# heracles-ec/heracles

Hardware: AMD Instinct MI355X
Metric: map->Cl pairs/sec + mixing-matrix build sec, nside=4096 lmax=6144 (higher is better)
Workload: dtype f64

## Files before the change

### heracles_amd/csrc/hx_fft_core.h

```cpp
#pragma once
#ifdef __HIPCC__
#include <hip/hip_runtime.h>
#define HX_HD __host__ __device__ __forceinline__
#else
#include <cmath>
#define HX_HD inline
struct double2 {
    double x, y;
};
#endif

namespace hxfft {

HX_HD double2 mk(double a, double b)
{
    double2 r;
    r.x = a;
    r.y = b;
    return r;
}
HX_HD double2 cadd(double2 a, double2 b) { return mk(a.x + b.x, a.y + b.y); }
HX_HD double2 csub(double2 a, double2 b) { return mk(a.x - b.x, a.y - b.y); }
HX_HD double2 cmul(double2 a, double2 b) { return mk(a.x * b.x - a.y * b.y, a.x * b.y + a.y * b.x); }
HX_HD double2 cmulc(double2 a, double2 b)
// ... 89 lines not shown
#endif
    for (int s = 0; s < K; ++s) {
        const int half = R >> (s + 1);
#ifdef __HIPCC__
#pragma unroll
#endif
        for (int b = 0; b < R; b += 2 * half)
#ifdef __HIPCC__
#pragma unroll
#endif
            for (int jj = 0; jj < half; ++jj) {
                const double2 u = x[b + jj], v = x[b + jj + half];
                x[b + jj] = cadd(u, v);
                x[b + jj + half] = rot16(csub(u, v), jj * (8 / half));
            }
    }
}
template <int K>
HX_HD void dit_inv_regs(double2 *x)
{
    constexpr int R = 1 << K;
#ifdef __HIPCC__
#pragma unroll
#endif
    for (int s = K - 1; s >= 0; --s) {
        const int half = R >> (s + 1);
#ifdef __HIPCC__
#pragma unroll
#endif
        for (int b = 0; b < R; b += 2 * half)
#ifdef __HIPCC__
#pragma unroll
#endif
            for (int jj = 0; jj < half; ++jj) {
                const double2 u = x[b + jj], v = rot16c(x[b + jj + half], jj * (8 / half));
                x[b + jj] = cadd(u, v);
                x[b + jj + half] = csub(u, v);
            }
    }
}

template <int K, class TW>
HX_HD void dif_pass_butterfly(double2 *buf, int i, int h, TW tw, int twN)
{
    constexpr int R = 1 << K;
    const int t = i & (h - 1), p = ((i - t) << K) + t;
    double2 x[R];
#ifdef __HIPCC__
#pragma unroll
#endif
    for (int j = 0; j < R; ++j) x[j] = buf[lds_slot(p + j * h)];
    dif_regs<K>(x);
    if (h > 1 && t) apply_tw_powers<K, false>(x, tw[t * (twN / (R * h))]);
#ifdef __HIPCC__
#pragma unroll
#endif
    for (int j = 0; j < R; ++j) buf[lds_slot(p + j * h)] = x[j];
}
template <int K, class TW>
HX_HD void dit_inv_pass_butterfly(double2 *buf, int i, int h, TW tw, int twN)
{
    constexpr int R = 1 << K;
    const int t = i & (h - 1), p = ((i - t) << K) + t;
    double2 x[R];
#ifdef __HIPCC__
#pragma unroll
#endif
    for (int j = 0; j < R; ++j) x[j] = buf[lds_slot(p + j * h)];
    if (h > 1 && t) apply_tw_powers<K, true>(x, tw[t * (twN / (R * h))]);
    dit_inv_regs<K>(x);
#ifdef __HIPCC__
#pragma unroll
#endif
    for (int j = 0; j < R; ++j) buf[lds_slot(p + j * h)] = x[j];
}

HX_HD int fft_sched_np(int p) { return p <= 0 ? 0 : (p - (p < 4 ? p : 4) + 3) / 4 + 1; }
HX_HD int fft_sched_k(int p, int a)
{
    const int last = p < 4 ? p : 4, rest = p - last, nfront = (rest + 3) / 4;
    return a < nfront ? rest / nfront + (a < rest % nfront ? 1 : 0) : last;
}

HX_HD double2 dif4_combine(double2 z0, double2 z1, double2 z2, double2 z3, int r)
{
    switch (r & 3) {
    case 0: return cadd(cadd(z0, z1), cadd(z2, z3));
    case 1: return cadd(csub(z0, z2), mul_mi(csub(z1, z3)));
    case 2: return cadd(csub(z0, z1), csub(z2, z3));
    default: return cadd(csub(z0, z2), mul_pi(csub(z1, z3)));
    }
}

HX_HD unsigned mod_by_inv(unsigned x, unsigned d, double inv)
{
    const int q = (int)((double)x * inv);
    int r = (int)x - q * (int)d;
    if (r < 0) r += (int)d;
    if (r >= (int)d) r -= (int)d;
    return (unsigned)r;
}

HX_HD unsigned load_phase_num(unsigned j, unsigned r, unsigned n, bool bluestein)
{
    unsigned long long q = (unsigned long long)j * r;
    if (bluestein) q += 2ull * j * j;
    return (unsigned)(q % (4ull * n));
}

HX_HD unsigned chirp_num(unsigned k, unsigned n)
{
    return (unsigned)(((unsigned long long)k * k) % (2ull * n));
}

}
```

### heracles_amd/csrc/hx_ring_fft.hip

```cpp
#include <algorithm>
#include <type_traits>

#include "hx_sht_common.h"


namespace hx {
__global__ __launch_bounds__(512) void k_init_bhat(PlanDev P, const int *__restrict__ rp_list,
                                                   double2 *__restrict__ bhat)
{
    extern __shared__ double2 buf[];
    const int rp = rp_list[blockIdx.x];
    const int n = P.nsub[rp];
    const int M = fft_size_for(n);
    for (int j = threadIdx.x; j < lds_fft_slots(M); j += blockDim.x) buf[j] = make_double2(0.0, 0.0);
    __syncthreads();
    for (int j = threadIdx.x; j < n; j += blockDim.x) {
        double2 c = expipi((double)chirp_num(j, n) / (double)n);
        buf[lds_slot(j)] = c;
        if (j) buf[lds_slot(M - j)] = c;
    }
    __syncthreads();
    lds_fft_dif(buf, M, P.tw, P.twN);
    double2 *out = bhat + P.bhat_off[rp];
    for (int e = threadIdx.x; e < M; e += blockDim.x) out[M >= 16 ? (e & 15) * (M >> 4) + (e >> 4) : e] = buf[lds_slot(e)];
}

__host__ __device__ inline int ring_ph_hi(int M) { return (4 * M) / 64 + 1; }
constexpr int RING_NTMAX = 512;
constexpr int RING_FB = 8;

template <int MODE, bool WSYM = false>
__global__ __launch_bounds__(RING_NTMAX) void k_ring_subdft(PlanDev P, const RingDesc *__restrict__ desc, int nrings, int nb, int Mclass,
                                                            const double *__restrict__ maps,
                                                            const double *__restrict__ pixw,
                                                            const double2 *__restrict__ zin,
                                                            double2 *__restrict__ Y, double *__restrict__ pixout = nullptr,
                                                            const double *__restrict__ ref = nullptr)
{
    extern __shared__ double2 buf[];
    __shared__ double2 tw_hi[TW_HI_MAX], tw_lo[64];
    double2 *ph_hi = buf + lds_fft_slots(Mclass), *ph_lo = ph_hi + ring_ph_hi(Mclass);
    const int nt = blockDim.x;
    const int nitems = ((nrings + 7) >> 3) * nb * 32;
    const TwFactored twf = load_tw_factored(tw_hi, tw_lo, P.tw, P.twN);
    int tid = threadIdx.x;
    auto ring_of = [&](int item) __attribute__((always_inline)) { return ((item >> 5) / nb) * 8 + (item & 7); };
    RingDesc cur = RingDesc{0, 0, 0, 1, 0};
    if ((int)blockIdx.x < nitems && ring_of(blockIdx.x) < nrings) cur = desc[ring_of(blockIdx.x)];
    for (int item = blockIdx.x; item < nitems; item += gridDim.x) {
        const int r = (item >> 3) & 3, set = item >> 5;
        const int ring = ring_of(item), c = set % nb;
        const int itn = item + gridDim.x, ringn = itn < nitems ? ring_of(itn) : nrings;
        const bool nextv = ringn < nrings;
        if (ring >= nrings) {
            if (nextv) cur = desc[ringn];
            continue;
        }
        const int n = cur.n;
        const long long sN = cur.sN, sS = cur.sS;
        const int M = fft_size_for(n), MP = lds_fft_slots(M);
        const bool blu = M != n;
        const int p = ilog2(M);
        const double2 *bh = P.bhat + cur.bhat_off;
        const double inv = 1.0 / M, inv4n = 0.25 / (double)n;
        asm volatile("; item" : "+v"(tid));
        const bool haveS = sS >= 0, odd = r & 1, pw = MODE == 0 && !WSYM && pixw != nullptr;
        constexpr bool wsym = MODE == 0 && WSYM;
        const double sg = (r & 2) ? -1.0 : 1.0;
        const double *mpN = maps + (long long)c * P.npix + sN, *mpS = maps + (long long)c * P.npix + (haveS ? sS : sN);
        const double *pwN = pixw + sN, *pwS = pixw + (haveS ? sS : sN);
        const double2 *zp = zin + (long long)c * P.ny + sN;
        double2 z[RING_FB][4];
        struct __attribute__((aligned(8))) Pair { double x, y; };
        Pair wsy[RING_FB / 2];
        auto load_batch_t = [&](auto WIDEC, int u0) __attribute__((always_inline)) {
            constexpr bool WIDE = decltype(WIDEC)::value;
#pragma unroll
            for (int u = 0; u < RING_FB; u += 2) {
                const int j = 2 * (tid + ((u0 + u) >> 1) * nt);
                const bool tail = WIDE && j == n - 1;
                const int jj = tail ? n - 2 : (j + 1 < n ? j : 0);
                wsy[u >> 1] = Pair{1.0, 1.0};
                if (MODE == 0 && wsym && WIDE) wsy[u >> 1] = *reinterpret_cast<const Pair *>(pwN + jj);
#pragma unroll
                for (int q = 0; q < 4; ++q) {
                    const int i = jj + q * n;
                    if (MODE == 0) {
                        Pair fn, fs;
                        if (WIDE) {
                            fn = *reinterpret_cast<const Pair *>(mpN + i);
                            fs = *reinterpret_cast<const Pair *>(mpS + i);
                            if (!wsym && pw) {
                                const Pair wn = *reinterpret_cast<const Pair *>(pwN + i), ws = *reinterpret_cast<const Pair *>(pwS + i);
                                fn.x *= wn.x; fn.y *= wn.y; fs.x *= ws.x; fs.y *= ws.y;
                            }
                            z[u][q] = make_double2(fn.x, fn.y);
                            z[u + 1][q] = make_double2(fs.x, fs.y);
                        } else {
                            fn.x = fn.y = mpN[q]; fs.x = fs.y = mpS[q];
                            if (pw || wsym) { fn.x *= pwN[q]; fs.x *= pwS[q]; fn.y = fn.x; fs.y = fs.x; }
                            z[u][q] = make_double2(fn.x, haveS ? fs.x : 0.0);
                            z[u + 1][q] = make_double2(fn.y, haveS ? fs.y : 0.0);
                        }
                    } else {
                        const int i0 = (j < n ? j : 0) + q * n, i1 = (j + 1 < n ? j + 1 : 0) + q * n;
                        z[u][q] = zp[i0];
                        z[u + 1][q] = zp[i1];
                    }
                }
            }
        };
        auto load_batch = [&](int u0) __attribute__((always_inline)) {
            if (n >= 2) load_batch_t(std::true_type{}, u0);
            else load_batch_t(std::false_type{}, u0);
        };
        auto finish_batch = [&](int u0) __attribute__((always_inline)) {
            if (MODE != 0 || n < 2) return;
#pragma unroll
            for (int u = 0; u < RING_FB; u += 2) {
                const int j = 2 * (tid + ((u0 + u) >> 1) * nt);
                const bool tail = j == n - 1;
                const Pair w = wsy[u >> 1];
#pragma unroll
                for (int q = 0; q < 4; ++q) {
                    const double2 rn = z[u][q], rs = z[u + 1][q];
                    const double nx = wsym ? rn.x * w.x : rn.x, ny = wsym ? rn.y * w.y : rn.y;
                    const double sx = wsym ? rs.x * w.x : rs.x, sy = wsym ? rs.y * w.y : rs.y;
                    z[u][q] = make_double2(tail ? ny : nx, haveS ? (tail ? sy : sx) : 0.0);
                    z[u + 1][q] = make_double2(ny, haveS ? sy : 0.0);
                }
            }
        };
        load_batch(0);
        int4 nd0 = make_int4(0, 0, 0, 0), nd1 = nd0;
        if (nextv) {
            const int4 *dp = reinterpret_cast<const int4 *>(desc + ringn) + (tid >> 30);
            nd0 = dp[0];
            nd1 = dp[1];
        }
        auto lds_barrier = []() __attribute__((always_inline)) {
            __builtin_amdgcn_s_waitcnt(0xc07f);
            __builtin_amdgcn_s_barrier();
        };
        lds_barrier();
        for (int a = tid; a <= (4 * n) >> 6; a += nt) ph_hi[a] = expipi(-(double)(a << 6) / (2.0 * n));
        if (tid < 64) ph_lo[tid] = expipi(-(double)tid / (2.0 * n));
        lds_barrier();
        auto phase = [&](unsigned q) __attribute__((always_inline)) {
            return cmul(ph_hi[q >> 6], ph_lo[q & 63]);
        };
        {
            for (int u0 = 0;;) {
                finish_batch(u0);
#pragma unroll
                for (int u = 0; u < RING_FB; ++u) {
                    const int j = 2 * (tid + ((u0 + u) >> 1) * nt) + (u & 1);
                    const double2 e0 = odd ? csub(z[u][0], z[u][2]) : cadd(z[u][0], z[u][2]);
                    const double2 e1 = odd ? mul_mi(csub(z[u][1], z[u][3])) : cadd(z[u][1], z[u][3]);
                    const double2 t = make_double2(fma(sg, e1.x, e0.x), fma(sg, e1.y, e0.y));
                    const unsigned jc = j < n ? j : 0;
                    const unsigned qn = blu ? mod_by_inv(jc * (unsigned)r + 2u * jc * jc, 4u * (unsigned)n, inv4n) : jc * (unsigned)r;
                    buf[j < n ? lds_slot(j) : MP - 1] = cmul(t, phase(qn));
                }
                u0 += RING_FB;
                if (u0 * nt >= n) break;
                load_batch(u0);
            }
            if (blu)
                for (int j = n + tid; j < M; j += nt) buf[lds_slot(j)] = make_double2(0.0, 0.0);
        }
        __syncthreads();
        if (nextv) {
            auto sc = [](int v) __attribute__((always_inline)) { return __builtin_amdgcn_readfirstlane(v); };
            cur.sN = ((long long)sc(nd0.y) << 32) | (unsigned)sc(nd0.x);
            cur.sS = ((long long)sc(nd0.w) << 32) | (unsigned)sc(nd0.z);
            cur.bhat_off = ((long long)sc(nd1.y) << 32) | (unsigned)sc(nd1.x);
            cur.n = sc(nd1.z);
            cur.rp = sc(nd1.w);
        }
        double2 *out = Y + (long long)c * P.ny + sN + (long long)r * n;
        double *pxN = nullptr, *pxS = nullptr;
        const double *rfN = nullptr, *rfS = nullptr;
        if (MODE == 1 && pixout) {
            pxN = pixout + (long long)c * P.npix + sN + r;
            pxS = pixout + (long long)c * P.npix + (haveS ? sS : sN) + r;
            if (ref) { rfN = ref + (long long)c * P.npix + sN + r; rfS = ref + (long long)c * P.npix + (haveS ? sS : sN) + r; }
        }
        const int kdrop0 = MODE == 0 ? (P.lmax - r) / 4 + 1 : n, kdrop1 = (4 * n - P.lmax - r + 3) / 4;
        auto emit = [&](int k, double2 v) __attribute__((always_inline)) {
            if (MODE == 0 && k >= kdrop0 && k < kdrop1) return;
            if (MODE == 1 && pxN) {
                double fn = v.x, fs = -v.y;
                if (rfN) { fn = rfN[4 * k] - fn; fs = rfS[4 * k] - fs; }
                pxN[4 * k] = fn;
                if (haveS) pxS[4 * k] = fs;
            } else {
                out[k] = v;
            }
        };
        if (!blu) {
            lds_fft_dif(buf, M, twf, P.twN);
            for (int k = tid; k < n; k += nt) emit(k, buf[lds_slot(bitrev(k, p))]);
            continue;
        }
        if (M >= 16) {
            double2 bq[16];
            const int nbf = M >> 4;
#pragma unroll
            for (int j = 0; j < 16; ++j) bq[j] = bh[j * nbf + (tid < nbf ? tid : 0)];
            lds_fft_dif(buf, M, twf, P.twN, tid, nt, true);
#pragma unroll 1
            for (int i = tid; i < nbf; i += nt) {
                double2 x[16];
#pragma unroll
                for (int j = 0; j < 16; ++j) x[j] = buf[lds_slot(16 * i) + j];
                dif_regs<4>(x);
#pragma unroll
                for (int j = 0; j < 16; ++j) {
                    x[j] = cmul(x[j], bq[j]);
                }
                if (i + nt < nbf) {
#pragma unroll
                    for (int j = 0; j < 16; ++j) bq[j] = bh[j * nbf + i + nt];
                }
                dit_inv_regs<4>(x);
#pragma unroll
                for (int j = 0; j < 16; ++j) buf[lds_slot(16 * i) + j] = x[j];
            }
            __syncthreads();
            lds_fft_dit_inv(buf, M, twf, P.twN, tid, nt, true);
        } else {
            lds_fft_dif(buf, M, twf, P.twN, tid, nt);
            for (int j = tid; j < M; j += nt) buf[lds_slot(j)] = cmul(buf[lds_slot(j)], bh[j]);
            __syncthreads();
            lds_fft_dit_inv(buf, M, twf, P.twN, tid, nt);
        }
        for (int k = tid; k < n; k += nt)
            emit(k, cscale(cmul(buf[lds_slot(k)], phase(2u * mod_by_inv((unsigned)k * (unsigned)k, 2u * (unsigned)n, 2.0 * inv4n))), inv));
    }
}

template <int MODE, bool WSYM = false>
__global__ __launch_bounds__(RING_NTMAX) void k_ring_pairfft(PlanDev P, const RingDesc *__restrict__ desc, int nrings, int nb, int M,
                                                             const double *__restrict__ maps, const double *__restrict__ pixw,
                                                             const double2 *__restrict__ zin, double2 *__restrict__ Y,
                                                             double *__restrict__ pixout = nullptr, const double *__restrict__ ref = nullptr)
{
    extern __shared__ double2 buf[];
    __shared__ double2 tw_hi[TW_HI_MAX], tw_lo[64];
    const int MP = lds_fft_slots(M), n = M, p = ilog2(M);
    double2 *ph_hi = buf + 2 * MP, *ph_lo = ph_hi + ring_ph_hi(M);
    const int nt = blockDim.x, nh = nt >> 1;
    const int nitems = ((nrings + 7) >> 3) * nb * 16;
    const TwFactored twf = load_tw_factored(tw_hi, tw_lo, P.tw, P.twN);
    int tid = threadIdx.x;
    for (int a = tid; a <= (4 * n) >> 6; a += nt) ph_hi[a] = expipi(-(double)(a << 6) / (2.0 * n));
    if (tid < 64) ph_lo[tid] = expipi(-(double)tid / (2.0 * n));
    __syncthreads();
    auto phase = [&](unsigned q) __attribute__((always_inline)) { return cmul(ph_hi[q >> 6], ph_lo[q & 63]); };
    auto ring_of = [&](int item) __attribute__((always_inline)) { return ((item >> 4) / nb) * 8 + (item & 7); };
    auto comp_of = [&](int item) __attribute__((always_inline)) { return (item >> 4) % nb; };
    RingDesc cur = RingDesc{0, 0, 0, 1, 0};
    if ((int)blockIdx.x < nitems && ring_of(blockIdx.x) < nrings) cur = desc[ring_of(blockIdx.x)];
    struct __attribute__((aligned(8))) Pair { double x, y; };
    double2 z[RING_FB][4];
    Pair wsy[RING_FB / 2];
    const bool pw = MODE == 0 && !WSYM && pixw != nullptr;
    constexpr bool wsym = MODE == 0 && WSYM;
    auto request = [&](auto U0C, const RingDesc &d, int c) __attribute__((always_inline)) {
        constexpr int U0 = decltype(U0C)::value;
        const bool hS = d.sS >= 0;
        const double *mpN = maps + (long long)c * P.npix + d.sN, *mpS = maps + (long long)c * P.npix + (hS ? d.sS : d.sN);
        const double *pwN = pixw + d.sN, *pwS = pixw + (hS ? d.sS : d.sN);
        const double2 *zp = zin + (long long)c * P.ny + d.sN;
#pragma unroll
        for (int u = U0; u < U0 + RING_FB / 2; u += 2) {
            const int j = 2 * (tid + (u >> 1) * nt), jj = j + 1 < n ? j : 0;
            wsy[u >> 1] = Pair{1.0, 1.0};
            if (MODE == 0 && wsym) wsy[u >> 1] = *reinterpret_cast<const Pair *>(pwN + jj);
#pragma unroll
            for (int q = 0; q < 4; ++q) {
                const int i = jj + q * n;
                if (MODE == 0) {
                    Pair fn = *reinterpret_cast<const Pair *>(mpN + i), fs = *reinterpret_cast<const Pair *>(mpS + i);
                    if (!wsym && pw) {
                        const Pair wn = *reinterpret_cast<const Pair *>(pwN + i), ws = *reinterpret_cast<const Pair *>(pwS + i);
                        fn.x *= wn.x; fn.y *= wn.y; fs.x *= ws.x; fs.y *= ws.y;
                    }
                    z[u][q] = make_double2(fn.x, fn.y);
                    z[u + 1][q] = make_double2(fs.x, fs.y);
                } else {
                    z[u][q] = zp[i];
                    z[u + 1][q] = zp[i + 1];
                }
            }
        }
    };
    auto finish = [&](bool hS) __attribute__((always_inline)) {
        if (MODE != 0) return;
#pragma unroll
        for (int u = 0; u < RING_FB; u += 2) {
            const Pair w = wsy[u >> 1];
#pragma unroll
            for (int q = 0; q < 4; ++q) {
                const double2 rn = z[u][q], rs = z[u + 1][q];
                const double nx = wsym ? rn.x * w.x : rn.x, ny = wsym ? rn.y * w.y : rn.y;
                const double sx = wsym ? rs.x * w.x : rs.x, sy = wsym ? rs.y * w.y : rs.y;
                z[u][q] = make_double2(nx, hS ? sx : 0.0);
                z[u + 1][q] = make_double2(ny, hS ? sy : 0.0);
            }
        }
    };
    using H0 = std::integral_constant<int, 0>;
// ... 144 lines not shown
            *o = add ? cadd(*o, v) : v;
        }
    };
    auto input = [&](int r, int j) __attribute__((always_inline)) {
        const double2 t = dif4_combine(z_at(j, 0), z_at(j, 1), z_at(j, 2), z_at(j, 3), r);
        const unsigned qn = load_phase_num(j, r, n, !plain);
        return qn ? cmul(t, expipi(-(double)qn / (2.0 * n))) : t;
    };
    for (int r = 0; r < 4; ++r) {
        if (plain) {
            __syncthreads();
#pragma unroll 4
            for (int u = 0; u < SPLIT_JMAX; ++u) {
                const int j = threadIdx.x + u * blockDim.x;
                if (j < n) buf[lds_slot(j)] = input(r, j);
            }
            __syncthreads();
            lds_fft_dif(buf, n, twf, P.twN);
            const int pbits = ilog2(n);
            for (int k = threadIdx.x; k < n; k += blockDim.x) emit(r, k, buf[lds_slot(bitrev(k, pbits))], false);
            continue;
        }
        for (int half = 0; half < 2; ++half) {
            __syncthreads();
#pragma unroll 4
            for (int u = 0; u < SPLIT_JMAX; ++u) {
                const int j = threadIdx.x + u * blockDim.x;
                if (j < C) {
                    double2 v = make_double2(0.0, 0.0);
                    if (j < n) {
                        v = input(r, j);
                        if (half) v = cmul(v, twf[j]);
                    }
                    buf[lds_slot(j)] = v;
                }
            }
            __syncthreads();
            lds_fft_dif(buf, C, twf, P.twN);
            for (int j = threadIdx.x; j < C; j += blockDim.x) buf[lds_slot(j)] = cmul(buf[lds_slot(j)], bh[half * C + j]);
            __syncthreads();
            lds_fft_dit_inv(buf, C, twf, P.twN);
#pragma unroll 4
            for (int u = 0; u < SPLIT_JMAX; ++u) {
                const int k = threadIdx.x + u * blockDim.x;
                if (k < n) {
                    double2 y = buf[lds_slot(k)];
                    if (half) y = cmulc(y, twf[k]);
                    emit(r, k, cscale(cmul(y, expipi(-(double)chirp_num(k, n) / (double)n)), inv), half != 0);
                }
            }
        }
    }
}

__global__ __launch_bounds__(256) void k_pixw_symmetry(PlanDev P, const double *__restrict__ pixw, int *__restrict__ flag)
{
    const int rp = blockIdx.x, n = P.nsub[rp];
    const long long sN = P.startN[rp], sS = P.startS[rp];
    bool ok = true;
    for (int j = threadIdx.x; j < n; j += blockDim.x) {
        const double w = pixw[sN + j];
#pragma unroll
        for (int q = 1; q < 4; ++q) ok = ok && pixw[sN + j + (long long)q * n] == w;
        if (sS >= 0) {
#pragma unroll
            for (int q = 0; q < 4; ++q) ok = ok && pixw[sS + j + (long long)q * n] == w;
        }
    }
    if (!ok) *flag = 0;
}

}

using namespace hx;

static int g_lds_fft_cap = 8192;
extern "C" int hx_set_max_lds_fft(int points)
{
    if (points < 16 || points > 8192 || (points & (points - 1))) return fail(HX_ERR_ARG, "hx_set_max_lds_fft: a power of two in [16, 8192]");
    g_lds_fft_cap = points;
    return HX_OK;
}

static size_t ring_class_lds(int M, bool pair) { return ((pair ? 2 : 1) * (size_t)lds_fft_slots(M) + ring_ph_hi(M) + 64) * sizeof(double2); }

static bool ring_class_is_pair(int n, int M, int cap) { return M == n && M >= 16 && M <= cap && ring_class_lds(M, true) + 4096 <= 160 * 1024; }

int hx::ring_fft_plan_init(hx_plan *pl, const std::vector<int> &nsub, const std::vector<long long> &sN, const std::vector<long long> &sS)
{
    const int cap = g_lds_fft_cap;
    std::map<std::pair<int, int>, std::vector<int>> byM;
    bool plain_beyond_cap = false;
    for (int rp = pl->nrp - 1; rp >= 0; --rp) {
        const int M = fft_size_for(nsub[rp]);
        byM[{M, ring_class_is_pair(nsub[rp], M, cap) ? -1 : 0}].push_back(rp);
        plain_beyond_cap = plain_beyond_cap || (M > cap && M == nsub[rp]);
    }
    const int maxM = byM.rbegin()->first.first;
    if (maxM > 2 * cap || plain_beyond_cap) return fail(HX_ERR_UNSUPPORTED, "hx_plan_create: nside=%d needs an in-LDS FFT of %d points (limit %d, %d for Bluestein rings); unsupported", pl->nside, maxM, cap, 2 * cap);
    pl->fft_cap = cap;
    pl->lds_fft = (size_t)lds_fft_slots(std::min(maxM, cap)) * sizeof(double2);
    for (auto it = byM.rbegin(); it != byM.rend(); ++it) {
        pl->fft_classes.push_back({it->first.first, (int)pl->h_fft_rp_list.size(), (int)it->second.size(), it->first.second});
        pl->h_fft_rp_list.insert(pl->h_fft_rp_list.end(), it->second.begin(), it->second.end());
    }
    HX_TRY(upload(pl->fft_rp_list, pl->h_fft_rp_list));
    std::vector<long long> boff(pl->nrp, -1);
    std::vector<int> blu_list, blu_split;
    long long btot = 0;
    std::map<int, long long> off_of_n;
    for (int rp = 0; rp < pl->nrp; ++rp) {
        int n = nsub[rp], M = fft_size_for(n);
        if (M == n) continue;
        auto it = off_of_n.find(n);
        if (it == off_of_n.end()) {
            it = off_of_n.emplace(n, btot).first;
            btot += M;
            (M > cap ? blu_split : blu_list).push_back(rp);
        }
        boff[rp] = it->second;
    }
    HX_TRY(upload(pl->bhat_off, boff));
    std::vector<RingDesc> desc;
    for (int rp : pl->h_fft_rp_list) desc.push_back(RingDesc{sN[rp], sS[rp], boff[rp], nsub[rp], rp});
    HX_TRY(upload(pl->fft_desc, desc));
    HX_TRY(pl->bhat.alloc(sizeof(double2) * std::max<long long>(btot, 1)));
    const void *const init_kernels[] = {(const void *)k_init_bhat, (const void *)k_init_bhat_split};
    const void *const ring_kernels[] = {(const void *)k_ring_subdft<0, false>,  (const void *)k_ring_subdft<0, true>,  (const void *)k_ring_subdft<1, false>,
                                        (const void *)k_ring_pairfft<0, false>, (const void *)k_ring_pairfft<0, true>, (const void *)k_ring_pairfft<1, false>,
                                        (const void *)k_ring_subdft_split<0>,   (const void *)k_ring_subdft_split<1>};
    for (const void *k : init_kernels) (void)hipFuncSetAttribute(k, hipFuncAttributeMaxDynamicSharedMemorySize, 160 * 1024);
    for (const void *k : ring_kernels) (void)hipFuncSetAttribute(k, hipFuncAttributeMaxDynamicSharedMemorySize, 156 * 1024);
    HX_HIP(hipGetLastError());
    hipStream_t st = rt().stream;
    if (!blu_list.empty()) {
        DevBuf d_list;
        HX_TRY(upload(d_list, blu_list));
        hipLaunchKernelGGL(k_init_bhat, dim3((unsigned)blu_list.size()), dim3(512), pl->lds_fft, st, pl->dev(),
                           d_list.as<int>(), pl->bhat.as<double2>());
        (void)hipStreamSynchronize(st);
    }
    if (!blu_split.empty()) {
        DevBuf d_list;
        HX_TRY(upload(d_list, blu_split));
        hipLaunchKernelGGL(k_init_bhat_split, dim3((unsigned)blu_split.size()), dim3(std::min(512, std::max(64, cap / 16))), (size_t)lds_fft_slots(cap) * sizeof(double2), st,
                           pl->dev(), d_list.as<int>(), cap, pl->bhat.as<double2>());
        (void)hipStreamSynchronize(st);
    }
    return HX_OK;
}

struct RingIO { const double *maps, *pixw; const double2 *zin; double2 *Y; double *pixout; const double *ref; };

template <auto KERNEL>
static void launch_ring_class(hx_plan *pl, const hx_plan::FftClass &c, int nb, const RingIO &io)
{
    const int k = c.big < 0 ? 2 : 1;
    const int threads = std::min(RING_NTMAX, k * std::max(64, c.M / 16));
    const size_t lds = ring_class_lds(c.M, k == 2);
    const int per_cu = (int)std::max<size_t>(1, std::min<size_t>(512 / threads, (160 * 1024) / (lds + 3 * 1024 + 256)));
    const long long items = ((long long)c.count + 7) / 8 * nb * (32 / k);
    const unsigned groups = (unsigned)std::min<long long>(items, (long long)rt().cus * per_cu);
    hipLaunchKernelGGL(KERNEL, dim3(groups), dim3(threads), lds, rt().stream, pl->dev(), pl->fft_desc.as<RingDesc>() + c.first, c.count, nb, c.M, io.maps, io.pixw, io.zin, io.Y, io.pixout, io.ref);
}

template <int MODE, bool WSYM>
static int launch_subdft_classes(hx_plan *pl, int nb, const RingIO &io, int rp_lo = 0, int rp_hi = 0x7fffffff)
{
    for (const auto &cls : pl->fft_classes) {
        hx_plan::FftClass c = cls;
        if (rp_lo > 0 || rp_hi < pl->nrp) {
            const int *b = pl->h_fft_rp_list.data() + cls.first, *e = b + cls.count;
            const int *x = std::lower_bound(b, e, rp_hi, [](int rp, int lim) { return rp >= lim; });
            const int *y = std::lower_bound(b, e, rp_lo, [](int rp, int lim) { return rp >= lim; });
            c.first = cls.first + (int)(x - b);
            c.count = (int)(y - x);
            if (c.count <= 0) continue;
        }
        if (c.big < 0)
            launch_ring_class<k_ring_pairfft<MODE, WSYM>>(pl, c, nb, io);
        else if (c.M > pl->fft_cap) {
            const int C = pl->fft_cap, threads = std::min(512, std::max(64, C / SPLIT_JMAX));
            hipLaunchKernelGGL(k_ring_subdft_split<MODE>, dim3(1, c.count, nb), dim3(threads), (size_t)lds_fft_slots(C) * sizeof(double2), rt().stream,
                               pl->dev(), pl->fft_rp_list.as<int>() + c.first, C, io.maps, io.pixw, io.zin, io.Y, io.pixout, io.ref);
        } else
            launch_ring_class<k_ring_subdft<MODE, WSYM>>(pl, c, nb, io);
    }
    HX_HIP(hipGetLastError());
    return HX_OK;
}

int hx::launch_ring_subdft_maps(hx_plan *pl, int nb, const double *d_maps, const double *d_pw, double2 *Y, int rp_lo, int rp_hi)
{
    ProfScope ps("ring_fft");
    if (d_pw && pl->pw_checked != d_pw) HX_TRY(classify_pixel_weights(pl, d_pw));
    const RingIO io = {d_maps, d_pw, nullptr, Y, nullptr, nullptr};
    return d_pw && pl->pw_mode == 2 ? launch_subdft_classes<0, true>(pl, nb, io, rp_lo, rp_hi) : launch_subdft_classes<0, false>(pl, nb, io, rp_lo, rp_hi);
}

int hx::launch_ring_subdft_spectra(hx_plan *pl, int nc, const double2 *zin, double *pixout, const double *ref)
// ... 19 lines not shown
```

### heracles_amd/csrc/hx_sht_common.h

```cpp
#pragma once
#include <map>
#include <vector>

#include "hx_common.h"
#include "hx_fft_core.h"

namespace hx {

typedef double double4_t __attribute__((ext_vector_type(4)));

constexpr int LBLK = 32;
constexpr int NCOL = 16;
constexpr int TABLE_PAD = 512;
constexpr int NGMAX = 2;
constexpr int RBLK = 32;
constexpr double SC_BIG = 0x1p+300, SC_SMALL = 0x1p-300;
constexpr int SPIN_ANY = -1;

struct LegTask {
    int m;
    int rb0;
    int nrb;
    int pad;
    long long pout;
// ... 135 lines not shown
    double2 ph;
    long long i0, i1;
    int hasS;
};

__device__ inline void ring_modes_ns(const PlanDev &P, const double2 *__restrict__ Y, int c, int rp, int m,
                                     const RingAtM &r, double2 &FN, double2 &FS, int s = 0)
{
    if (P.nssrc) {
        const double4 v = P.nssrc[c][(long long)((m - P.ns_m0) / P.ns_ms) * P.nrp_pad + rp];
        FN = make_double2(v.x, v.y);
        FS = make_double2(v.z, v.w);
        return;
    }
    if (P.hsrc) {
        const double w = r.ph.x;
        const double2 *h = P.hsrc + (long long)c * P.hsrc_stride + (long long)m * P.hN;
        const double sg = ((m + s) & 1) ? -w : w;
        const double2 a = h[rp], b = h[P.hN - 1 - rp], cN = h[P.hN / 2 - 1 - rp], d = h[P.hN / 2 + rp];
        FN = make_double2(w * a.x + sg * b.x, w * a.y + sg * b.y);
        FS = make_double2(w * cN.x + sg * d.x, w * cN.y + sg * d.y);
        return;
    }
    const double2 *Yc = Y + (long long)c * P.ny;
    const double2 a = Yc[r.i0], b = cconj(Yc[r.i1]);
    const double2 xn = cscale(cadd(a, b), 0.5);
    const double2 xs = mul_mi(cscale(csub(a, b), 0.5));
    FN = cmul(xn, r.ph);
    FS = r.hasS ? cmul(xs, r.ph) : make_double2(0.0, 0.0);
}

__device__ inline RingAtM ring_at_m_of(const PlanDev &P, int r, int m, const double *__restrict__ rw)
{
    RingAtM q;
    const bool live = r < P.nrp;
    const double w = live ? (rw ? rw[r] : 1.0) * P.wnorm : 0.0;
    q.ph = make_double2(w, 0.0);
    q.i0 = q.i1 = 0;
    q.hasS = 0;
    if (live && !P.hsrc) {
        const int n = P.nsub[r], nphi = 4 * n;
        const int mm = m % nphi, mc = (nphi - mm) % nphi;
        q.i0 = P.startN[r] + (long long)(mm & 3) * n + (mm >> 2);
        q.i1 = P.startN[r] + (long long)(mc & 3) * n + (mc >> 2);
        if (P.shifted[r]) q.ph = cscale(expipi(-(double)(m % (2 * nphi)) / (double)nphi), w);
        q.hasS = P.startS[r] >= 0;
    }
    return q;
}

template <class TW>
__device__ __forceinline__ void lds_fft_pass_dif(double2 *buf, int M, int K, int h, int gt, int gn, TW tw, int twN)
{
    switch (K) {
    case 4:
_Pragma("unroll 1")
        for (int i = gt; i < (M >> 4); i += gn) dif_pass_butterfly<4>(buf, i, h, tw, twN); break;
    case 3:
_Pragma("unroll 1")
        for (int i = gt; i < (M >> 3); i += gn) dif_pass_butterfly<3>(buf, i, h, tw, twN); break;
    case 2:
_Pragma("unroll 1")
        for (int i = gt; i < (M >> 2); i += gn) dif_pass_butterfly<2>(buf, i, h, tw, twN); break;
    default: for (int i = gt; i < (M >> 1); i += gn) dif_pass_butterfly<1>(buf, i, h, tw, twN); break;
    }
}
template <class TW>
__device__ __forceinline__ void lds_fft_pass_dit_inv(double2 *buf, int M, int K, int h, int gt, int gn, TW tw, int twN)
{
    switch (K) {
    case 4:
_Pragma("unroll 1")
        for (int i = gt; i < (M >> 4); i += gn) dit_inv_pass_butterfly<4>(buf, i, h, tw, twN); break;
    case 3:
_Pragma("unroll 1")
        for (int i = gt; i < (M >> 3); i += gn) dit_inv_pass_butterfly<3>(buf, i, h, tw, twN); break;
    case 2:
_Pragma("unroll 1")
        for (int i = gt; i < (M >> 2); i += gn) dit_inv_pass_butterfly<2>(buf, i, h, tw, twN); break;
    default: for (int i = gt; i < (M >> 1); i += gn) dit_inv_pass_butterfly<1>(buf, i, h, tw, twN); break;
    }
}
template <class TW>
__device__ __forceinline__ void lds_fft_dif(double2 *buf, int M, TW tw, int twN, int gt, int gn, bool skip_last = false)
{
    const int p = ilog2(M), np = fft_sched_np(p);
    int h = M;
    for (int a = 0; a < np - (skip_last ? 1 : 0); ++a) {
        const int K = fft_sched_k(p, a);
        h >>= K;
        lds_fft_pass_dif(buf, M, K, h, gt, gn, tw, twN);
        __syncthreads();
    }
}
template <class TW>
__device__ __forceinline__ void lds_fft_dit_inv(double2 *buf, int M, TW tw, int twN, int gt, int gn, bool skip_first = false)
{
    const int p = ilog2(M), np = fft_sched_np(p);
    int h = 1;
    for (int a = np - 1; a >= 0; --a) {
        const int K = fft_sched_k(p, a);
        if (!(skip_first && a == np - 1)) {
            lds_fft_pass_dit_inv(buf, M, K, h, gt, gn, tw, twN);
            __syncthreads();
        }
        h <<= K;
    }
}
template <class TW>
__device__ __forceinline__ void lds_fft_dif(double2 *buf, int M, TW tw, int twN) { lds_fft_dif(buf, M, tw, twN, (int)threadIdx.x, (int)blockDim.x); }
template <class TW>
__device__ __forceinline__ void lds_fft_dit_inv(double2 *buf, int M, TW tw, int twN) { lds_fft_dit_inv(buf, M, tw, twN, (int)threadIdx.x, (int)blockDim.x); }

constexpr int TW_HI_MAX = 128;
__device__ inline TwFactored load_tw_factored(double2 *hi, double2 *lo, const double2 *__restrict__ tw, int twN)
{
    for (int i = threadIdx.x; i < (twN >= 128 ? twN / 128 : 1); i += blockDim.x) hi[i] = tw[i * 64];
    for (int i = threadIdx.x; i < 64; i += blockDim.x) lo[i] = tw[i];
    TwFactored f;
    f.hi = hi;
    f.lo = lo;
    return f;
}

#endif

template <class T>
inline int upload(DevBuf &b, const std::vector<T> &v)
{
    HX_TRY(b.alloc(sizeof(T) * (v.size() > 0 ? v.size() : 1)));
    if (!v.empty()) HX_HIP(hipMemcpy(b.p, v.data(), sizeof(T) * v.size(), hipMemcpyHostToDevice));
    return HX_OK;
}

}

struct hx_plan {
    int nside = 0, lmax = 0, max_comp = 0;
    int nrp = 0, nrp_pad = 0, twN = 1;
    int fft_cap = 8192;
    int last_chunks = 0;
    int eqN = 0;
    double wnorm = 0.0;
    const double2 *hsrc = nullptr;
    long long hsrc_stride = 0;
    const double4 *const *nssrc = nullptr;
    int ns_m0 = 0;
    int m_lo = 0, m_hi = -1, m_step = 1;
    int leadin_resume = 1;
    long long leadin_cap = 0;
    long long npix = 0, ny = 0, nlm = 0;
    size_t lds_fft = 0;
    hx::DevBuf z, omz, sth, rwdef, nsub, shifted, startN, startS, bhat_off, tw, bhat, mfac, kfac2;
    std::vector<double> h_sth, h_z;
    std::vector<int> h_nsub;
    std::vector<long long> h_startN, h_startS;
    struct TaskSet {
        std::vector<hx::LegTask> tasks;
        std::vector<hx::MTasks> of_m;
        std::vector<long long> rows_before_m;
        std::vector<long long> arow;
        hx::DevBuf d_tasks, d_of_m, d_arow;
        hx::DevBuf d_leadin;
        bool leadin_skip = false;
    };
    struct SpinData {
        hx::DevBuf cn, al, kf;
        hx::DevBuf syn_mlim;
        hx::DevBuf syn_boff;
        std::map<int, TaskSet> tasks;
    };
    std::map<std::pair<int, bool>, SpinData> spins;
    struct FftClass { int M, first, count, big; };
    std::vector<FftClass> fft_classes;
    hx::DevBuf fft_rp_list;
    hx::DevBuf fft_desc;
    std::vector<int> h_fft_rp_list;
    hx::DevBuf Y, F, partial, d_dbg, resid_maps, pw_sym;
    hx::DevBuf syn_tab;
    const double *pw_checked = nullptr;
    int pw_mode = 0;
    static constexpr int NSTAGE = 3;
    hx::DevBuf stage[NSTAGE];
    hipEvent_t stage_done[NSTAGE] = {nullptr, nullptr, nullptr};
    static constexpr int NUNIT_EV = 4;
    hipEvent_t unit_up[NUNIT_EV] = {nullptr, nullptr, nullptr, nullptr};
    hx::PlanDev dev() const;
};

namespace hx {
hx_plan *plan_create_equiangular(int N, int lmax);
// ... 50 lines not shown
```

Baseline: 433.0.

## Use mixed-radix 3/5/7 Bluestein padding sizes instead of power-of-two

Bluestein convolution lengths for non-power-of-two rings are now chosen as 5/8, 6/8 or 7/8 of the next power of two when that is large enough, rather than always the full power of two. This shrinks the padded FFT length. The forward and inverse transforms get an odd-radix (3, 5, 7) first or last pass, optionally fused with a few radix-2 stages, followed by the existing power-of-two block FFTs. Costs are extra twiddle tables in LDS, more code paths, and more registers in the fused odd-radix butterflies.

Result: no change. 432.7 (-0.1%).

```diff
diff --git a/heracles_amd/csrc/hx_fft_core.h b/heracles_amd/csrc/hx_fft_core.h
--- a/heracles_amd/csrc/hx_fft_core.h
+++ b/heracles_amd/csrc/hx_fft_core.h
@@ -195,6 +195,233 @@
     return a < nfront ? rest / nfront + (a < rest % nfront ? 1 : 0) : last;
 }
 
+HX_HD int bluestein_size(int n, int K)
+{
+    const int need = n + K - 1;
+    int P2 = 1;
+    while (P2 < need) P2 <<= 1;
+    if (P2 < 128) return P2;
+    if (5 * (P2 >> 3) >= need) return 5 * (P2 >> 3);
+    if (6 * (P2 >> 3) >= need) return 6 * (P2 >> 3);
+    if (7 * (P2 >> 3) >= need) return 7 * (P2 >> 3);
+    return P2;
+}
+HX_HD int ring_fft_len(int n) { return (n & (n - 1)) == 0 ? n : bluestein_size(n, n); }
+HX_HD int fft_odd_factor(int M)
+{
+    while (M > 1 && !(M & 1)) M >>= 1;
+    return M > 0 ? M : 1;
+}
+
+template <int P>
+HX_HD double odd_cos(int k)
+{
+    if (P == 3) return -0.5;
+    if (P == 5) return k == 1 ? 0.30901699437494742410 : -0.80901699437494742410;
+    return k == 1 ? 0.62348980185873353053 : k == 2 ? -0.22252093395631440429 : -0.90096886790241912624;
+}
+template <int P>
+HX_HD double odd_sin(int k)
+{
+    if (P == 3) return 0.86602540378443864676;
+    if (P == 5) return k == 1 ? 0.95105651629515357212 : 0.58778525229247312917;
+    return k == 1 ? 0.78183148246802980871 : k == 2 ? 0.97492791218182360702 : 0.43388373911755812048;
+}
+template <int P, bool INV>
+HX_HD void dft_odd_regs(double2 *x)
+{
+    constexpr int H = (P - 1) / 2;
+    double2 s[H], d[H];
+#ifdef __HIPCC__
+#pragma unroll
+#endif
+    for (int a = 1; a <= H; ++a) {
+        s[a - 1] = cadd(x[a], x[P - a]);
+        d[a - 1] = csub(x[a], x[P - a]);
+    }
+    const double2 x0 = x[0];
+#ifdef __HIPCC__
+#pragma unroll
+#endif
+    for (int a = 1; a <= H; ++a) x[0] = cadd(x[0], s[a - 1]);
+#ifdef __HIPCC__
+#pragma unroll
+#endif
+    for (int b = 1; b <= H; ++b) {
+        double2 A = x0, B = mk(0.0, 0.0);
+#ifdef __HIPCC__
+#pragma unroll
+#endif
+        for (int a = 1; a <= H; ++a) {
+            const int k = (a * b) % P, kk = k <= H ? k : P - k;
+            const double c = odd_cos<P>(kk), sn = k <= H ? odd_sin<P>(kk) : -odd_sin<P>(kk);
+            A = mk(fma(c, s[a - 1].x, A.x), fma(c, s[a - 1].y, A.y));
+            B = mk(fma(sn, d[a - 1].x, B.x), fma(sn, d[a - 1].y, B.y));
+        }
+        x[INV ? P - b : b] = cadd(A, mul_mi(B));
+        x[INV ? b : P - b] = cadd(A, mul_pi(B));
+    }
+}
+template <int P, class TWM>
+HX_HD void mixed_first_pass_butterfly(double2 *buf, int t, int L, int nin, TWM twm)
+{
+    double2 x[P];
+#ifdef __HIPCC__
+#pragma unroll
+#endif
+    for (int a = 0; a < P; ++a) x[a] = t + a * L < nin ? buf[lds_slot(t + a * L)] : mk(0.0, 0.0);
+    dft_odd_regs<P, false>(x);
+    if (t) {
+        const double2 w = twm[t];
+        double2 wb = w;
+#ifdef __HIPCC__
+#pragma unroll
+#endif
+        for (int b = 1; b < P; ++b) {
+            x[b] = cmul(x[b], wb);
+            if (b + 1 < P) wb = cmul(wb, w);
+        }
+    }
+#ifdef __HIPCC__
+#pragma unroll
+#endif
+    for (int b = 0; b < P; ++b) buf[lds_slot(t + b * L)] = x[b];
+}
+template <int P, class TWM>
+HX_HD void mixed_last_pass_inv_butterfly(double2 *buf, int t, int L, int nout, TWM twm)
+{
+    double2 x[P];
+#ifdef __HIPCC__
+#pragma unroll
+#endif
+    for (int b = 0; b < P; ++b) x[b] = buf[lds_slot(t + b * L)];
+    if (t) {
+        const double2 w = twm[t];
+        double2 wb = w;
+#ifdef __HIPCC__
+#pragma unroll
+#endif
+        for (int b = 1; b < P; ++b) {
+            x[b] = cmulc(x[b], wb);
+            if (b + 1 < P) wb = cmul(wb, w);
+        }
+    }
+    dft_odd_regs<P, true>(x);
+#ifdef __HIPCC__
+#pragma unroll
+#endif
+    for (int a = 0; a < P; ++a)
+        if (t + a * L < nout) buf[lds_slot(t + a * L)] = x[a];
+}
+HX_HD int mixed_fuse_q(int podd, int L)
+{
+    const int lb = ilog2(L), q = lb > 8 ? lb - 8 : 0, qmax = podd == 3 ? 3 : podd == 5 ? 2 : 1;
+    return q < qmax ? q : qmax;
+}
+template <int P, int Q, class TWM, class TW>
+HX_HD void mixed_first_fused_butterfly(double2 *buf, int t, int L, int nin, TWM twm, TW tw, int twN)
+{
+    constexpr int R = 1 << Q;
+    const int h = L >> Q;
+    double2 x[R][P];
+#ifdef __HIPCC__
+#pragma unroll
+#endif
+    for (int c = 0; c < R; ++c) {
+        const int tc = t + c * h;
+#ifdef __HIPCC__
+#pragma unroll
+#endif
+        for (int a = 0; a < P; ++a) x[c][a] = tc + a * L < nin ? buf[lds_slot(tc + a * L)] : mk(0.0, 0.0);
+        dft_odd_regs<P, false>(x[c]);
+        if (tc) {
+            const double2 w = twm[tc];
+            double2 wb = w;
+#ifdef __HIPCC__
+#pragma unroll
+#endif
+            for (int b = 1; b < P; ++b) {
+                x[c][b] = cmul(x[c][b], wb);
+                if (b + 1 < P) wb = cmul(wb, w);
+            }
+        }
+    }
+    const double2 w = tw[t * (twN / L)];
+#ifdef __HIPCC__
+#pragma unroll
+#endif
+    for (int b = 0; b < P; ++b) {
+        double2 y[R];
+#ifdef __HIPCC__
+#pragma unroll
+#endif
+        for (int c = 0; c < R; ++c) y[c] = x[c][b];
+        dif_regs<Q>(y);
+        if (t) apply_tw_powers<Q, false>(y, w);
+#ifdef __HIPCC__
+#pragma unroll
+#endif
+        for (int j = 0; j < R; ++j) buf[lds_slot(b * L + t + j * h)] = y[j];
+    }
+}
+template <int P, int Q, class TWM, class TW>
+HX_HD void mixed_last_fused_inv_butterfly(double2 *buf, int t, int L, int nout, TWM twm, TW tw, int twN)
+{
+    constexpr int R = 1 << Q;
+    const int h = L >> Q;
+    double2 x[R][P];
+    const double2 w = tw[t * (twN / L)];
+#ifdef __HIPCC__
+#pragma unroll
+#endif
+    for (int b = 0; b < P; ++b) {
+        double2 y[R];
+#ifdef __HIPCC__
+#pragma unroll
+#endif
+        for (int j = 0; j < R; ++j) y[j] = buf[lds_slot(b * L + t + j * h)];
+        if (t) apply_tw_powers<Q, true>(y, w);
+        dit_inv_regs<Q>(y);
+#ifdef __HIPCC__
+#pragma unroll
+#endif
+        for (int c = 0; c < R; ++c) x[c][b] = y[c];
+    }
+#ifdef __HIPCC__
+#pragma unroll
+#endif
+    for (int c = 0; c < R; ++c) {
+        const int tc = t + c * h;
+        if (tc) {
+            const double2 wm = twm[tc];
+            double2 wb = wm;
+#ifdef __HIPCC__
+#pragma unroll
+#endif
+            for (int b = 1; b < P; ++b) {
+                x[c][b] = cmulc(x[c][b], wb);
+                if (b + 1 < P) wb = cmul(wb, wm);
+            }
+        }
+        dft_odd_regs<P, true>(x[c]);
+#ifdef __HIPCC__
+#pragma unroll
+#endif
+        for (int a = 0; a < P; ++a)
+            if (tc + a * L < nout) buf[lds_slot(tc + a * L)] = x[c][a];
+    }
+}
+struct TwMixed {
+    const double2 *hi, *lo;
+    HX_HD double2 operator[](int t) const { return cmul(hi[t >> 4], lo[t & 15]); }
+};
+HX_HD int tw_mixed_hi(int Mclass) { return Mclass / 64 + 1; }
+HX_HD int ring_ph_hi(int M) { return (4 * M) / 64 + 1; }
+HX_HD int ring_lds_entries(int Mclass, bool pair)
+{
+    return (pair ? 2 : 1) * lds_fft_slots(Mclass) + ring_ph_hi(Mclass) + 64 + (pair ? 0 : tw_mixed_hi(Mclass) + 16);
+}
+
 HX_HD double2 dif4_combine(double2 z0, double2 z1, double2 z2, double2 z3, int r)
 {
     switch (r & 3) {
diff --git a/heracles_amd/csrc/hx_ring_fft.hip b/heracles_amd/csrc/hx_ring_fft.hip
--- a/heracles_amd/csrc/hx_ring_fft.hip
+++ b/heracles_amd/csrc/hx_ring_fft.hip
@@ -5,13 +5,18 @@
 
 
 namespace hx {
+struct TwMixedDirect {
+    double m2inv;
+    __device__ double2 operator[](int t) const { return expipi((double)t * m2inv); }
+};
+
 __global__ __launch_bounds__(512) void k_init_bhat(PlanDev P, const int *__restrict__ rp_list,
                                                    double2 *__restrict__ bhat)
 {
     extern __shared__ double2 buf[];
     const int rp = rp_list[blockIdx.x];
     const int n = P.nsub[rp];
-    const int M = fft_size_for(n);
+    const int M = bluestein_size(n, n), podd = fft_odd_factor(M), L = M / podd;
     for (int j = threadIdx.x; j < lds_fft_slots(M); j += blockDim.x) buf[j] = make_double2(0.0, 0.0);
     __syncthreads();
     for (int j = threadIdx.x; j < n; j += blockDim.x) {
@@ -20,12 +25,13 @@
         if (j) buf[lds_slot(M - j)] = c;
     }
     __syncthreads();
-    lds_fft_dif(buf, M, P.tw, P.twN);
+    const int fq = podd > 1 ? mixed_fuse_q(podd, L) : 0;
+    if (podd > 1) lds_fft_mixed_first(buf, podd, L, fq, M, (int)threadIdx.x, (int)blockDim.x, TwMixedDirect{-2.0 / (double)M}, P.tw, P.twN);
+    lds_fft_dif_blocks(buf, M, L >> fq, P.tw, P.twN, (int)threadIdx.x, (int)blockDim.x);
     double2 *out = bhat + P.bhat_off[rp];
     for (int e = threadIdx.x; e < M; e += blockDim.x) out[M >= 16 ? (e & 15) * (M >> 4) + (e >> 4) : e] = buf[lds_slot(e)];
 }
 
-__host__ __device__ inline int ring_ph_hi(int M) { return (4 * M) / 64 + 1; }
 constexpr int RING_NTMAX = 512;
 constexpr int RING_FB = 8;
 
@@ -40,6 +46,8 @@
     extern __shared__ double2 buf[];
     __shared__ double2 tw_hi[TW_HI_MAX], tw_lo[64];
     double2 *ph_hi = buf + lds_fft_slots(Mclass), *ph_lo = ph_hi + ring_ph_hi(Mclass);
+    double2 *mx_hi = ph_lo + 64, *mx_lo = mx_hi + tw_mixed_hi(Mclass);
+    const TwMixed twm = {mx_hi, mx_lo};
     const int nt = blockDim.x;
     const int nitems = ((nrings + 7) >> 3) * nb * 32;
     const TwFactored twf = load_tw_factored(tw_hi, tw_lo, P.tw, P.twN);
@@ -58,8 +66,10 @@
         }
         const int n = cur.n;
         const long long sN = cur.sN, sS = cur.sS;
-        const int M = fft_size_for(n), MP = lds_fft_slots(M);
+        const int M = ring_fft_len(n), MP = lds_fft_slots(M);
         const bool blu = M != n;
+        const int podd = blu ? fft_odd_factor(M) : 1, L = M / podd;
+        const int fq = podd > 1 ? mixed_fuse_q(podd, L) : 0;
         const int p = ilog2(M);
         const double2 *bh = P.bhat + cur.bhat_off;
         const double inv = 1.0 / M, inv4n = 0.25 / (double)n;
@@ -145,6 +155,10 @@
         lds_barrier();
         for (int a = tid; a <= (4 * n) >> 6; a += nt) ph_hi[a] = expipi(-(double)(a << 6) / (2.0 * n));
         if (tid < 64) ph_lo[tid] = expipi(-(double)tid / (2.0 * n));
+        if (podd > 1) {
+            for (int a = tid; a <= L >> 4; a += nt) mx_hi[a] = expipi(-2.0 * (double)(a << 4) / (double)M);
+            if (tid < 16) mx_lo[tid] = expipi(-2.0 * (double)tid / (double)M);
+        }
         lds_barrier();
         auto phase = [&](unsigned q) __attribute__((always_inline)) {
             return cmul(ph_hi[q >> 6], ph_lo[q & 63]);
@@ -166,7 +180,7 @@
                 if (u0 * nt >= n) break;
                 load_batch(u0);
             }
-            if (blu)
+            if (blu && podd == 1)
                 for (int j = n + tid; j < M; j += nt) buf[lds_slot(j)] = make_double2(0.0, 0.0);
         }
         __syncthreads();
@@ -206,9 +220,10 @@
         if (M >= 16) {
             double2 bq[16];
             const int nbf = M >> 4;
+            if (podd > 1) lds_fft_mixed_first(buf, podd, L, fq, n, tid, nt, twm, twf, P.twN);
 #pragma unroll
             for (int j = 0; j < 16; ++j) bq[j] = bh[j * nbf + (tid < nbf ? tid : 0)];
-            lds_fft_dif(buf, M, twf, P.twN, tid, nt, true);
+            lds_fft_dif_blocks(buf, M, L >> fq, twf, P.twN, tid, nt, true);
 #pragma unroll 1
             for (int i = tid; i < nbf; i += nt) {
                 double2 x[16];
@@ -228,7 +243,8 @@
                 for (int j = 0; j < 16; ++j) buf[lds_slot(16 * i) + j] = x[j];
             }
             __syncthreads();
-            lds_fft_dit_inv(buf, M, twf, P.twN, tid, nt, true);
+            lds_fft_dit_inv_blocks(buf, M, L >> fq, twf, P.twN, tid, nt, true);
+            if (podd > 1) lds_fft_mixed_last_inv(buf, podd, L, fq, n, tid, nt, twm, twf, P.twN);
         } else {
             lds_fft_dif(buf, M, twf, P.twN, tid, nt);
             for (int j = tid; j < M; j += nt) buf[lds_slot(j)] = cmul(buf[lds_slot(j)], bh[j]);
@@ -539,7 +555,7 @@
     return HX_OK;
 }
 
-static size_t ring_class_lds(int M, bool pair) { return ((pair ? 2 : 1) * (size_t)lds_fft_slots(M) + ring_ph_hi(M) + 64) * sizeof(double2); }
+static size_t ring_class_lds(int M, bool pair) { return (size_t)ring_lds_entries(M, pair) * sizeof(double2); }
 
 static bool ring_class_is_pair(int n, int M, int cap) { return M == n && M >= 16 && M <= cap && ring_class_lds(M, true) + 4096 <= 160 * 1024; }
 
@@ -572,7 +588,7 @@
         auto it = off_of_n.find(n);
         if (it == off_of_n.end()) {
             it = off_of_n.emplace(n, btot).first;
-            btot += M;
+            btot += M > cap ? M : bluestein_size(n, n);
             (M > cap ? blu_split : blu_list).push_back(rp);
         }
         boff[rp] = it->second;
diff --git a/heracles_amd/csrc/hx_sht_common.h b/heracles_amd/csrc/hx_sht_common.h
--- a/heracles_amd/csrc/hx_sht_common.h
+++ b/heracles_amd/csrc/hx_sht_common.h
@@ -241,10 +241,10 @@
     }
 }
 template <class TW>
-__device__ __forceinline__ void lds_fft_dif(double2 *buf, int M, TW tw, int twN, int gt, int gn, bool skip_last = false)
-{
-    const int p = ilog2(M), np = fft_sched_np(p);
-    int h = M;
+__device__ __forceinline__ void lds_fft_dif_blocks(double2 *buf, int M, int L, TW tw, int twN, int gt, int gn, bool skip_last = false)
+{
+    const int p = ilog2(L), np = fft_sched_np(p);
+    int h = L;
     for (int a = 0; a < np - (skip_last ? 1 : 0); ++a) {
         const int K = fft_sched_k(p, a);
         h >>= K;
@@ -253,9 +253,9 @@
     }
 }
 template <class TW>
-__device__ __forceinline__ void lds_fft_dit_inv(double2 *buf, int M, TW tw, int twN, int gt, int gn, bool skip_first = false)
-{
-    const int p = ilog2(M), np = fft_sched_np(p);
+__device__ __forceinline__ void lds_fft_dit_inv_blocks(double2 *buf, int M, int L, TW tw, int twN, int gt, int gn, bool skip_first = false)
+{
+    const int p = ilog2(L), np = fft_sched_np(p);
     int h = 1;
     for (int a = np - 1; a >= 0; --a) {
         const int K = fft_sched_k(p, a);
@@ -266,6 +266,60 @@
         h <<= K;
     }
 }
+template <class TW>
+__device__ __forceinline__ void lds_fft_dif(double2 *buf, int M, TW tw, int twN, int gt, int gn, bool skip_last = false) { lds_fft_dif_blocks(buf, M, M, tw, twN, gt, gn, skip_last); }
+template <class TW>
+__device__ __forceinline__ void lds_fft_dit_inv(double2 *buf, int M, TW tw, int twN, int gt, int gn, bool skip_first = false) { lds_fft_dit_inv_blocks(buf, M, M, tw, twN, gt, gn, skip_first); }
+#define HX_MIXED_CASE(P, Q, FN, NLIM)                                                                       \
+    case 4 * P + Q:                                                                                         \
+_Pragma("unroll 1")                                                                                         \
+        for (int t = gt; t < (L >> Q); t += gn) FN<P, Q>(buf, t, L, NLIM, twm, tw, twN);                    \
+        break;
+template <class TWM, class TW>
+__device__ __forceinline__ void lds_fft_mixed_first(double2 *buf, int podd, int L, int q, int nin, int gt, int gn, TWM twm, TW tw, int twN)
+{
+    switch (4 * podd + q) {
+    HX_MIXED_CASE(3, 1, mixed_first_fused_butterfly, nin)
+    HX_MIXED_CASE(3, 2, mixed_first_fused_butterfly, nin)
+    HX_MIXED_CASE(3, 3, mixed_first_fused_butterfly, nin)
+    HX_MIXED_CASE(5, 1, mixed_first_fused_butterfly, nin)
+    HX_MIXED_CASE(5, 2, mixed_first_fused_butterfly, nin)
+    HX_MIXED_CASE(7, 1, mixed_first_fused_butterfly, nin)
+    case 4 * 3:
+_Pragma("unroll 1")
+        for (int t = gt; t < L; t += gn) mixed_first_pass_butterfly<3>(buf, t, L, nin, twm); break;
+    case 4 * 5:
+_Pragma("unroll 1")
+        for (int t = gt; t < L; t += gn) mixed_first_pass_butterfly<5>(buf, t, L, nin, twm); break;
+    default:
+_Pragma("unroll 1")
+        for (int t = gt; t < L; t += gn) mixed_first_pass_butterfly<7>(buf, t, L, nin, twm); break;
+    }
+    __syncthreads();
+}
+template <class TWM, class TW>
+__device__ __forceinline__ void lds_fft_mixed_last_inv(double2 *buf, int podd, int L, int q, int nout, int gt, int gn, TWM twm, TW tw, int twN)
+{
+    switch (4 * podd + q) {
+    HX_MIXED_CASE(3, 1, mixed_last_fused_inv_butterfly, nout)
+    HX_MIXED_CASE(3, 2, mixed_last_fused_inv_butterfly, nout)
+    HX_MIXED_CASE(3, 3, mixed_last_fused_inv_butterfly, nout)
+    HX_MIXED_CASE(5, 1, mixed_last_fused_inv_butterfly, nout)
+    HX_MIXED_CASE(5, 2, mixed_last_fused_inv_butterfly, nout)
+    HX_MIXED_CASE(7, 1, mixed_last_fused_inv_butterfly, nout)
+    case 4 * 3:
+_Pragma("unroll 1")
+        for (int t = gt; t < L; t += gn) mixed_last_pass_inv_butterfly<3>(buf, t, L, nout, twm); break;
+    case 4 * 5:
+_Pragma("unroll 1")
+        for (int t = gt; t < L; t += gn) mixed_last_pass_inv_butterfly<5>(buf, t, L, nout, twm); break;
+    default:
+_Pragma("unroll 1")
+        for (int t = gt; t < L; t += gn) mixed_last_pass_inv_butterfly<7>(buf, t, L, nout, twm); break;
+    }
+    __syncthreads();
+}
+#undef HX_MIXED_CASE
 template <class TW>
 __device__ __forceinline__ void lds_fft_dif(double2 *buf, int M, TW tw, int twN) { lds_fft_dif(buf, M, tw, twN, (int)threadIdx.x, (int)blockDim.x); }
 template <class TW>
```
